# hdelan/MSc-HPC-Final-Project

Hardware: AMD Instinct MI355X
Metric: lanczos_iterations_per_sec (higher is better)
Workload: dtype f64

## Files before the change

### msc-hpc-final-project_amd/csrc/lzx_api.hip

```cpp
#include <algorithm>
#include <atomic>
#include <chrono>
#include <cmath>
#include <cstdlib>
#include <cstring>
#include <string>
#include <thread>

#include "lzx_internal.h"

static thread_local std::string g_err;

void lzx_set_error(const char *fmt, ...)
{
    char buf[1024];
    va_list ap;
    va_start(ap, fmt);
    vsnprintf(buf, sizeof buf, fmt, ap);
    va_end(ap);
    g_err = buf;
}

extern "C" const char *lzx_last_error(void) { return g_err.c_str(); }

// ... 155 lines not shown
}

extern "C" int lzx_test_set_shape(lzx_handle c, const char *name, int64_t value)
{
    if (!c || !name) LZX_FAIL(LZX_ERR_ARG, "lzx_test_set_shape: bad argument");
    if (c->d_row_ptr) LZX_FAIL(LZX_ERR_STATE, "shapes must be set before the graph is handed over");
    const Option *o = find_option(name, OPT_SHAPE);
    if (!o) LZX_FAIL(LZX_ERR_ARG, "lzx_test_set_shape: unknown shape '%s'", name);
    store_option(c, *o, value);
    return LZX_OK;
}

extern "C" int lzx_test_get_shape(lzx_handle c, const char *name, int64_t *value)
{
    if (!c || !name || !value) LZX_FAIL(LZX_ERR_ARG, "lzx_test_get_shape: bad argument");
    if (!strcmp(name, "gather_items_dealt")) *value = c->pb ? c->pb_n_static : 0;
    else if (!strcmp(name, "gather_items_drawn")) *value = c->pb ? c->pb_n_dyn : 0;
    else if (!strcmp(name, "gather_workgroups")) *value = c->pb ? c->pb_gather_grid : 0;
    else if (!strcmp(name, "placement_tried")) *value = c->place_tried;
    else if (!strcmp(name, "placement_kept")) *value = c->place_kept;
    else if (!strcmp(name, "start_vector_was_constant")) *value = c->x0_was_constant ? 1 : 0;
    else if (!strcmp(name, "finish_deferrable")) *value = c->pb && c->pb_defer_ok ? 1 : 0;
    else if (!strcmp(name, "finish_launched")) *value = c->pb && c->pb_finish_grid ? 1 : 0;
    else if (!strncmp(name, "placement_us_", 13) && name[13] >= '0' && name[13] <= '7' && !name[14]) *value = (int64_t)(c->place_ms[name[13] - '0'] * 1e3f);
    else LZX_FAIL(LZX_ERR_ARG, "lzx_test_get_shape: unknown shape '%s'", name);
    return LZX_OK;
}

extern "C" int lzx_test_allreduce_latency(lzx_handle c, uint32_t reps, double *us_each)
{
    if (!c || !us_each || reps == 0) LZX_FAIL(LZX_ERR_ARG, "lzx_test_allreduce_latency: bad argument");
    if (c->comm_kind < 2 || !lzx_exchanges(c)) LZX_FAIL(LZX_ERR_STATE, "lzx_test_allreduce_latency: needs a one-process-per-rank communicator");
    std::vector<lzx_ctx *> cs(1, c);
    LZX_HIP(hipSetDevice(c->device));
    LZX_HIP(hipMemsetAsync(c->d_scal, 0, sizeof(double) * 2, c->stream));
    for (u32 i = 0; i < 5; ++i) LZX_TRY(lzx_comm_allreduce_sum(cs, 0, 2));
    LZX_HIP(hipEventRecord(c->ev_a, c->stream));
    for (u32 i = 0; i < reps; ++i) LZX_TRY(lzx_comm_allreduce_sum(cs, 0, 2));
    LZX_HIP(hipEventRecord(c->ev_b, c->stream));
    LZX_HIP(hipStreamSynchronize(c->stream));
    LZX_TRY(lzx_comm_ipc_check(c));
    float ms = 0.f;
    LZX_HIP(hipEventElapsedTime(&ms, c->ev_a, c->ev_b));
    *us_each = (double)ms * 1e3 / reps;
    return LZX_OK;
}
// ... 1181 lines not shown
```

### msc-hpc-final-project_amd/csrc/lzx_internal.h

```cpp
#pragma once

#include <hip/hip_runtime.h>

#include <algorithm>
#include <chrono>
#include <cmath>
#include <cstdarg>
#include <cstdint>
#include <cstdio>
#include <vector>

#include "lzx.h"

typedef uint32_t u32;
typedef uint64_t u64;

void lzx_set_error(const char *fmt, ...);

#define LZX_HIP(call)                                                                          \
    do {                                                                                       \
        hipError_t e_ = (call);                                                                \
        if (e_ != hipSuccess) {                                                                \
            lzx_set_error("%s:%d: %s -> %s", __FILE__, __LINE__, #call, hipGetErrorString(e_)); \
            return (e_ == hipErrorOutOfMemory) ? LZX_ERR_NOMEM : LZX_ERR_HIP;                   \
// ... 154 lines not shown
    u64 long_elems = 0;
    u32 *d_long_cols = nullptr;
    u64 *d_item_beg = nullptr;
    u32 *d_item_len = nullptr;
    u32 *d_item_first = nullptr;
    double *d_long_partial = nullptr;

    bool pb = false;
    u32 hub_real = 0;
    u64 pb_entries = 0;
    u32 pb_nr = 0;
    u32 pb_units = 0;
    uint16_t *d_pb_lcol = nullptr;
    u32 *d_pb_dst = nullptr;
    uint16_t *d_pb_lrow = nullptr;
    double *d_pb_val = nullptr;
    u32 *d_pb_unit = nullptr;
    u32 *d_pb_row0 = nullptr;
    u32 *d_pb_rep = nullptr;
    u32 *d_pb_beg = nullptr;
    u32 *d_pb_items = nullptr;
    u32 *d_pb_multi = nullptr;
    double *d_pb_part = nullptr;
    uint8_t *d_pb_long_multi = nullptr;
    int64_t pb_stamps_opt = -1;
    unsigned long long *d_pb_gstamps = nullptr;
    int64_t tie_sort_opt = -1;
    int64_t item_opt = -1;
    int64_t vec_per_cu_opt = -1;
    int64_t burst_opt = -1;
    int64_t deep_opt = -1;
    int64_t pb_order_opt = -1;
    int64_t pb_group_opt = -1;
    int64_t pb_group_force_opt = -1;
    int64_t pb_gwaves_opt = -1;
    u32 pb_gather_block = 512;
    u32 pb_n_items = 0, pb_n_multi = 0;
    u32 pb_gather_grid = 0, pb_finish_grid = 0;
    uint4 *d_pb_mrow = nullptr;
    u32 pb_multi_limit = 0;
    bool pb_defer_ok = false, pb_deferring = false;
    int64_t defer_opt = -1;
    double *d_pb_item_dot = nullptr;
    u32 pb_n_static = 0, pb_n_dyn = 0;
    u32 *d_pb_gcounter = nullptr;
    int64_t spmv_wgs_opt = -1;
// ... 318 lines not shown
```

### msc-hpc-final-project_amd/csrc/lzx_kernels.hip

```cpp
#include <type_traits>
#include <algorithm>
#include "lzx_internal.h"
#include "lzx_spmv_body.h"
#include "lzx_reduce.h"


template <int HUB, bool NT>
__global__ void __launch_bounds__(LZX_SPMV_BLOCK) k_spmv(const SpmvArgs a)
{
    spmv_body<HUB, NT>(a, blockIdx.x, gridDim.x);
}

__global__ void __launch_bounds__(LZX_VEC_BLOCK)
k_long_finish(const u32 *item_first, const double *long_partial, u32 n_long, const double *q_loc,
              double *v, double *partials)
{
    __shared__ double sh[4];
    const u32 r = blockIdx.x * LZX_VEC_BLOCK + threadIdx.x;
    double dot = 0.0;
    if (r < n_long) {
        double s = 0.0;
        for (u32 it = item_first[r]; it < item_first[r + 1]; ++it) s += long_partial[it];
        v[r] = s;
        dot = s * q_loc[r];
    }
    block_partial(dot, sh, partials);
}

__global__ void __launch_bounds__(LZX_VEC_BLOCK)
k_reduce(const double *partials, u32 np, double *out, int do_sqrt)
{
    __shared__ double sh[4];
    const double t = block_sum_fixed_256(partials, np, sh);
// ... 445 lines not shown
{
    const u32 need = (c->n_loc_pad / 2 + LZX_VEC_BLOCK - 1) / LZX_VEC_BLOCK;
    const u32 cap = (u32)c->cu_count * (c->vec_per_cu_opt > 0 ? (u32)c->vec_per_cu_opt : (c->n_loc_pad <= (4u << 20) ? 4u : 8u));
    return need < 1 ? 1 : (need < cap ? need : cap);
}

u32 lzx_spmv_partials(const lzx_ctx *c) { return c->spmv_grid + (c->pb ? 0 : c->fin_grid) + lzx_pb_partials(c) - (c->pb_deferring && c->pb_defer_ok ? c->pb_finish_grid : 0u); }

static LazyDeferred lazy_deferred(const lzx_ctx *c)
{
    LazyDeferred d;
    if (c->pb && c->pb_deferring && c->pb_defer_ok) {
        d.mrow = c->d_pb_mrow;
        d.limit = c->pb_multi_limit;
        d.part = c->d_pb_part;
        d.item_first = c->d_item_first;
        d.long_partial = c->d_long_partial;
        d.long_mode = c->d_pb_long_multi;
        d.n_long = c->n_long64;
    }
    return d;
}

template <int HUB, bool NT>
static int launch_spmv_t(lzx_ctx *c, const SpmvArgs &a, hipStream_t st)
{
    auto kern = k_spmv<HUB, NT>;
    LZX_HIP(hipFuncSetAttribute(reinterpret_cast<const void *>(kern),
                                hipFuncAttributeMaxDynamicSharedMemorySize, (int)c->spmv_lds));
    hipLaunchKernelGGL(kern, dim3(c->spmv_grid), dim3(LZX_SPMV_BLOCK), c->spmv_lds, st, a);
    return LZX_OK;
}

int lzx_launch_spmv(lzx_ctx *c, const SpmvLaunch &l)
{
    SpmvArgs a;
    a.sell_cols = c->d_sell_cols;
    a.slice_off = c->d_slice_off;
    a.slice_w = c->d_slice_w;
    const u32 live_slices = l.live_rows_only ? (c->rows_live > c->n_long64 ? (c->rows_live - c->n_long64) / LZX_SLICE : 0u) : c->n_slices;
    a.slice_perm = c->d_slice_perm;
    a.ns_w8 = c->ns_w8;
    a.ns_w4 = c->ns_w4;
    a.ns_w0 = (u32)(std::lower_bound(c->h_slice_w0.begin(), c->h_slice_w0.end(), live_slices) - c->h_slice_w0.begin());
    a.n_slices = c->ns_wide;
    if (c->ns_wide == c->n_slices) a.n_slices = std::min<u32>(c->n_slices, live_slices);
    if (!(c->phase_mask_opt & 2)) a.n_slices = a.ns_w8 = a.ns_w4 = a.ns_w0 = 0;
    a.row0 = c->n_long64;
    a.long_cols = c->d_long_cols;
    a.item_beg = c->d_item_beg;
// ... 19 lines not shown
    if (side) {
        LZX_HIP(hipEventRecord(c->ev_fork, c->stream));
        LZX_HIP(hipStreamWaitEvent(c->stream3, c->ev_fork, 0));
        hs = c->stream3;
    }
    bool fused = false;
    const bool fuse_chunked = c->pb && !side && l.chunk1_ready && c->codes16 && !nt && !c->trace && c->fuse_opt != 0 && c->fuse_opt != 1 &&
                              lzx_pb_can_fuse(c);
    if (fuse_chunked) {
        LZX_TRY(lzx_pb_launch(c, l.x, l.q_loc, l.v, pb_partials, l.chunk1_ready, nullptr, 3, &a, c->spmv_grid, &fused));
        if (fused) {
            LZX_HIP(hipGetLastError());
            return LZX_OK;
        }
        LZX_FAIL(LZX_ERR_STATE, "fused launch was refused");
    }
    if (scatter_first) {
        if (c->trace) LZX_HIP(hipEventRecord(c->trace_ev[2], c->stream));
        const bool fuse = c->codes16 && !nt && !c->trace && c->fuse_opt != 0 && lzx_pb_can_fuse(c);
        LZX_TRY(lzx_pb_launch(c, l.x, l.q_loc, l.v, pb_partials, l.chunk1_ready, nullptr, 1, fuse ? &a : nullptr, c->spmv_grid, &fused));
    }
    if (c->trace) LZX_HIP(hipEventRecord(c->trace_ev[0], c->stream));
    if (fused) {
    } else if (c->codes16) {
        if (nt) LZX_TRY((launch_spmv_t<2, true>(c, a, hs)));
        else    LZX_TRY((launch_spmv_t<2, false>(c, a, hs)));
    } else if (c->hub > 0) {
        if (nt) LZX_TRY((launch_spmv_t<1, true>(c, a, hs)));
        else    LZX_TRY((launch_spmv_t<1, false>(c, a, hs)));
    } else {
        if (nt) LZX_TRY((launch_spmv_t<0, true>(c, a, hs)));
        else    LZX_TRY((launch_spmv_t<0, false>(c, a, hs)));
    }
    if (c->trace) LZX_HIP(hipEventRecord(c->trace_ev[1], c->stream));
    if (c->fin_grid > 0 && !c->pb) {
        hipLaunchKernelGGL(k_long_finish, dim3(c->fin_grid), dim3(LZX_VEC_BLOCK), 0, hs,
                           c->d_item_first, c->d_long_partial, c->n_long64, l.q_loc, l.v,
                           l.partials + c->spmv_grid);
    }
    LZX_HIP(hipGetLastError());
    if (c->trace && !scatter_first) LZX_HIP(hipEventRecord(c->trace_ev[2], c->stream));
    if (side) LZX_HIP(hipEventRecord(c->ev_join, c->stream3));
    if (scatter_first) {
        if (c->trace) LZX_HIP(hipEventRecord(c->trace_ev[5], c->stream));
        LZX_TRY(lzx_pb_launch(c, l.x, l.q_loc, l.v, pb_partials, nullptr, nullptr, 2));
    } else {
// ... 251 lines not shown
```

### msc-hpc-final-project_amd/csrc/lzx_pb.hip

```cpp
#include <hipcub/hipcub.hpp>

#include <algorithm>
#include <cstdlib>
#include <queue>
#include <utility>

#include "lzx_internal.h"
#include "lzx_spmv_body.h"
#include "lzx_pb_shared.h"

namespace {

constexpr u32 KEY_LCOL_BITS = 15, KEY_LROW_SHIFT = KEY_LCOL_BITS, KEY_CBAND_SHIFT = KEY_LROW_SHIFT + 10, KEY_RBAND_SHIFT = KEY_CBAND_SHIFT + 16;
constexpr u32 KEY_LCOL_MASK = (1u << KEY_LCOL_BITS) - 1u;
__device__ __forceinline__ u64 pack_key(u32 rband, u32 cband, u32 lrow, u32 lcol)
{
    return ((u64)rband << KEY_RBAND_SHIFT) | ((u64)cband << KEY_CBAND_SHIFT) | ((u64)lrow << KEY_LROW_SHIFT) | (u64)lcol;
}

__global__ void __launch_bounds__(64)
k_pb_emit(const u64 *row_ptr, const u32 *col_idx, const u32 *code_of_old, const u32 *old_of_local,
          const u32 *deg_local, const u32 *nh_off, u32 n_rows, u32 hub, const u32 *band_row0, u32 nr, u32 cb, u64 *keys)
{
    const u32 lane = threadIdx.x;
    for (u32 l = blockIdx.x; l < n_rows; l += gridDim.x) {
        const u32 d = deg_local[l];
        u32 lo = 0, hi = nr;
        while (hi - lo > 1) {
            const u32 mid = (lo + hi) >> 1;
            if (band_row0[mid] <= l) lo = mid; else hi = mid;
        }
        const u32 R = lo, lrow = l - band_row0[lo];
// ... 481 lines not shown
                    out[1] = hi;
                }
            }
        }
        }
    }
}

template <u32 CB, bool SCAN, bool NTC>
__global__ void __launch_bounds__(1024)
k_pb_scatter(const u32 *unit, const uint4 *scode, const u32 *sbase, const uint2 *q_lcol, const u32 *q_dst,
             const double *__restrict__ x, u64 xlen, double *val)
{
    pb_scatter_body<CB, SCAN, NTC>(unit, scode, sbase, q_lcol, q_dst, x, xlen, val, blockIdx.x);
}

template <u32 CB, bool SCAN, bool NTC>
__global__ void __launch_bounds__(1024)
k_pb_scatter_spmv(const u32 *unit, u32 n_units, const uint4 *scode, const u32 *sbase, const uint2 *q_lcol, const u32 *q_dst,
                  const double *__restrict__ x, u64 xlen, double *val, const SpmvArgs a, const u32 spmv_first)
{
    const u32 spmv_blocks = gridDim.x - n_units;
    if (spmv_first) {
        if (blockIdx.x < spmv_blocks) spmv_body<2, false>(a, blockIdx.x, spmv_blocks);
        else pb_scatter_body<CB, SCAN, NTC>(unit, scode, sbase, q_lcol, q_dst, x, xlen, val, blockIdx.x - spmv_blocks);
        return;
    }
    if (blockIdx.x < n_units) pb_scatter_body<CB, SCAN, NTC>(unit, scode, sbase, q_lcol, q_dst, x, xlen, val, blockIdx.x);
    else spmv_body<2, false>(a, blockIdx.x - n_units, spmv_blocks);
}

template <bool NT>
__device__ __forceinline__ double2 gld_val2(const double *p)
{
    typedef double d2v __attribute__((ext_vector_type(2)));
    const d2v t = NT ? __builtin_nontemporal_load(reinterpret_cast<const d2v *>(p)) : *reinterpret_cast<const d2v *>(p);
    return make_double2(t.x, t.y);
}
template <bool NT>
__device__ __forceinline__ u32 gld_slot2(const uint16_t *p)
{
    return NT ? __builtin_nontemporal_load(reinterpret_cast<const u32 *>(p)) : *reinterpret_cast<const u32 *>(p);
}

__device__ __forceinline__ void tile_add2(double *ytile, u32 lane, u32 sv, double ax, double ay)
{
    const u32 s0 = sv & 0xffffu, s1 = sv >> 16;
    const u32 spare = LZX_PB_RB + lane;
    atomicAdd(&ytile[min(s0, spare)], ax);
    atomicAdd(&ytile[min(s1, spare)], ay);
    if (__ballot((s0 | s1) >= 1024u)) {
        u32 r = 1;
// ... 69 lines not shown
        ticket = uni(*ltick);
        if (ticket >= n_dyn) {
            if (tid == 0 && ticket == n_dyn + gridDim.x - 1) *counter = 0u;
            break;
        }
        base = n_static + ticket; stride = 0; limit = base + 1; nrounds = 1;
        __syncthreads();
    }
    for (u32 t = tid; t < nrounds * WAVES; t += LZX_PB_GATHER_BLOCK) {
        const u32 r = t / WAVES, w = t % WAVES;
        const u32 it = base + r * stride;
        u32 *o = lrec + (size_t)t * 8;
        uint4 item = make_uint4(0u, 0u, 0u, LZX_PB_ITEM_NONE);
        if (it < limit) item = items[it];
        o[5] = item.w;
        o[6] = 0u;
        o[7] = 1u;
        if (item.w == LZX_PB_ITEM_GROUP) {
            const u32 y = item.y, split = y <= 1u ? 8u : y <= 2u ? 4u : y <= 4u ? 2u : 1u;
            o[7] = split;
            if (w < y * split) {
                const u32 R = item.x + w % y;
                const u32 r0 = band_row0[R];
                o[0] = band_beg[R]; o[1] = band_beg[R + 1]; o[2] = r0; o[3] = band_row0[R + 1] - r0; o[4] = band_rep[R]; o[6] = 1u + (w / y) + (y << 8);
            }
        } else if (item.w != LZX_PB_ITEM_NONE) {
            const u32 R = item.x;
            const u32 r0 = band_row0[R];
            o[0] = item.y; o[1] = item.z; o[2] = r0; o[3] = band_row0[R + 1] - r0; o[4] = band_rep[R];
            o[6] = 1u + (item.y == band_beg[R] ? 2u : 0u);
        }
    }
    __syncthreads();
    const double dot_static = dot;
    if (dyn) dot = 0.0;
    for (u32 rr = 0; rr < nrounds && base + rr * stride < limit; ++rr) {
        const u32 *rec = lrec + ((size_t)rr * WAVES + wv) * 8;
        const u32 r_beg = uni(rec[0]), r_end = uni(rec[1]), r_row0 = uni(rec[2]), r_rows = uni(rec[3]), r_rep = uni(rec[4]);
        const u32 item_w = uni(rec[5]), r_live = uni(rec[6]), r_split = uni(rec[7]);
        if (item_w == LZX_PB_ITEM_NONE) continue;
        if (item_w == LZX_PB_ITEM_GROUP) {
            __syncthreads();
            const u32 part = r_live ? (r_live & 0xffu) - 1u : 0u, gy = r_live >> 8;
            if (r_live) {
                const u32 rows = r_rows, rep = r_rep;
                const u32 beg = r_beg, end = r_end;
                const u32 slots = rows * rep;
                for (u32 j = lane; j < slots; j += 64) ytile[j] = 0.0;
                __builtin_amdgcn_wave_barrier();
                if (STAMP && part == 0) { ++n_it; n_vals += end - beg; }
                GSTAMP(t_zero);
                const u32 blocks = (end - beg) / 128u;
                u32 kb = part;
                for (; kb + 7 * r_split < blocks; kb += 8 * r_split) {
                    double2 av[8];
                    u32 sv[8];
#pragma unroll
                    for (int u = 0; u < 8; ++u) {
                        const u32 p = beg + (kb + u * r_split) * 128u + lane * 2;
                        av[u] = gld_val2<NT>(val + p);
                        sv[u] = NOSLOT ? (lane * 2u) | ((lane * 2u + 1u) << 16) : gld_slot2<NT>(lslot + p);
                    }
#pragma unroll
                    for (int u = 0; u < 8; ++u) tile_add2(ytile, lane, sv[u], av[u].x, av[u].y);
                }
                {
// ... 33 lines not shown
                        u32 h8[8];
#pragma unroll
                        for (int u = 0; u < 8; ++u) {
                            h8[u] = ((i + u * 64) * 2654435761u + r_row0 * 40503u) >> 7;
                            t8[u] = xt[h8[u] & 0x1ffffu];
                        }
#pragma unroll
                        for (int u = 0; u < 8; ++u)
                            if (i + u * 64 < probe_l2g) tile_add1(ytile, lane, (h8[u] >> 17) % slots, t8[u]);
                    }
                }
#endif
                __builtin_amdgcn_wave_barrier();
                GSTAMP(t_stream);
            }
            if (r_split > 1u) __syncthreads();
            if (r_live && part == 0u) {
                const u32 row0 = r_row0, rows = r_rows, rep = r_rep;
                for (u32 j0 = lane; j0 < rows; j0 += 256) {
                    double vv[4], qq[4];
#pragma unroll
                    for (int u = 0; u < 4; ++u) {
                        const u32 j = j0 + u * 64;
                        vv[u] = j < rows ? v[row0 + j] : 0.0;
                        qq[u] = j < rows ? q_loc[row0 + j] : 0.0;
                    }
#pragma unroll
                    for (int u = 0; u < 4; ++u) {
                        const u32 j = j0 + u * 64;
                        if (j < rows) {
                            double y = 0.0;
                            for (u32 pt = 0; pt < r_split; ++pt)
                                for (u32 t = 0; t < rep; ++t) y += ytile[(size_t)pt * gy * TILE + j * rep + t];
                            v[row0 + j] = vv[u] + y;
                            dot += y * qq[u];
                        }
                    }
                }
                close_split_rows(row0, rows, lane, 64u, dot, 0u);
                GSTAMP(t_fold);
            }
            continue;
        }
        const u32 beg = r_beg, end = r_end;
        if (STAMP) { ++n_it; n_vals += end - beg; }
        const u32 row0 = r_row0, rows = r_rows;
        if (rows == 1) {
            double acc = 0.0;
            u32 i = beg + tid;
            for (; i + 7 * LZX_PB_GATHER_BLOCK < end; i += 8 * LZX_PB_GATHER_BLOCK) {
                double a[8];
#pragma unroll
                for (int u = 0; u < 8; ++u) a[u] = val[i + u * LZX_PB_GATHER_BLOCK];
#pragma unroll
                for (int u = 0; u < 8; ++u) acc += a[u];
            }
            for (; i < end; i += LZX_PB_GATHER_BLOCK) acc += val[i];
            acc = wave_sum_pb(acc);
            __syncthreads();
            if (lane == 0) wsum[wv] = acc;
            __syncthreads();
            if (tid == 0) {
                double t = 0.0;
                for (u32 w = 0; w < WAVES; ++w) t += wsum[w];
                if (item_w == 0xffffffffu) {
                    double vr = v[row0] + t;
                    dot += t * q_loc[row0];
                    if (row0 < n_long && long_mode[row0] == 0) {
                        double sl = 0.0;
                        for (u32 it = item_first[row0]; it < item_first[row0 + 1]; ++it) sl += long_partial[it];
                        vr += sl;
                        dot += sl * q_loc[row0];
                    }
                    v[row0] = vr;
                } else {
                    part[item_w] = t;
                    dot += t * q_loc[row0];
                    if ((r_live & 2u) && row0 < n_long && long_mode[row0] == 1) {
                        double sl = 0.0;
                        for (u32 it = item_first[row0]; it < item_first[row0 + 1]; ++it) sl += long_partial[it];
                        dot += sl * q_loc[row0];
                    }
                }
            }
            continue;
        }
        const u32 rep = r_rep;
        const u32 slots = rows * rep;
        __syncthreads();
        for (u32 j = lane; j < slots; j += 64) ytile[j] = 0.0;
        __builtin_amdgcn_wave_barrier();
        GSTAMP(t_zero);
        const u32 blocks = (end - beg) / 128u;
        u32 kb = wv;
        for (; kb + 7 * WAVES < blocks; kb += 8 * WAVES) {
            double2 av[8];
            u32 sv[8];
#pragma unroll
            for (int u = 0; u < 8; ++u) {
// ... 4 lines not shown
#pragma unroll
            for (int u = 0; u < 8; ++u) tile_add2(ytile, lane, sv[u], av[u].x, av[u].y);
        }
        for (; kb < blocks; kb += WAVES) {
            const u32 p = beg + kb * 128u + lane * 2;
            const double2 a = gld_val2<NT>(val + p);
            const u32 s = NOSLOT ? (lane * 2u) | ((lane * 2u + 1u) << 16) : gld_slot2<NT>(lslot + p);
            tile_add2(ytile, lane, s, a.x, a.y);
        }
        if (wv == 0)
            for (u32 i0 = beg + blocks * 128u; i0 < end; i0 += 64) {
                const u32 i = i0 + lane;
                tile_add1(ytile, lane, i < end ? (u32)lslot[i] : 0u, i < end ? val[i] : 0.0);
            }
        GSTAMP(t_stream);
        __syncthreads();
        GSTAMP(t_bar);
        if (item_w == 0xffffffffu) {
            for (u32 j0 = tid; j0 < rows; j0 += 2 * LZX_PB_GATHER_BLOCK) {
                double vv[2], qq[2];
#pragma unroll
                for (int u = 0; u < 2; ++u) {
                    const u32 j = j0 + u * LZX_PB_GATHER_BLOCK;
                    vv[u] = j < rows ? v[row0 + j] : 0.0;
                    qq[u] = j < rows ? q_loc[row0 + j] : 0.0;
                }
#pragma unroll
                for (int u = 0; u < 2; ++u) {
                    const u32 j = j0 + u * LZX_PB_GATHER_BLOCK;
                    if (j < rows) {
                        double y = 0.0;
                        for (u32 w = 0; w < WAVES; ++w)
                            for (u32 t = 0; t < rep; ++t) y += lds[(size_t)w * TILE + j * rep + t];
                        v[row0 + j] = vv[u] + y;
                        dot += y * qq[u];
                    }
                }
            }
            close_split_rows(row0, rows, tid, LZX_PB_GATHER_BLOCK, dot, 0u);
        } else {
            for (u32 j = tid; j < rows; j += LZX_PB_GATHER_BLOCK) {
                double y = 0.0;
                for (u32 w = 0; w < WAVES; ++w)
                    for (u32 t = 0; t < rep; ++t) y += lds[(size_t)w * TILE + j * rep + t];
                part[item_w + j] = y;
                dot += y * q_loc[row0 + j];
            }
            if (r_live & 2u) close_split_rows(row0, rows, tid, LZX_PB_GATHER_BLOCK, dot, 1u);
        }
        GSTAMP(t_fold);
    }
    if (dyn) {
        const double idot = wave_sum_pb(dot);
        dot = dot_static;
        __syncthreads();
        if (lane == 0) wsum[wv] = idot;
        __syncthreads();
        if (tid == 0) {
            double t = 0.0;
            for (u32 w = 0; w < WAVES; ++w) t += wsum[w];
            item_dot[ticket] = t;
        }
    } else {
        it0 += MAXR * gridDim.x;
    }
    }
    if (STAMP && tid == 0) {
        unsigned long long *o = stamps + 8 * (size_t)blockIdx.x;
        o[0] = t_start; o[1] = wall_clock64(); o[2] = t_zero; o[3] = t_stream; o[4] = t_bar; o[5] = t_fold;
// ... 102 lines not shown
    LZX_HIP(hipStreamSynchronize(c->stream));
    return rc;
}

void lzx_pb_release(lzx_ctx *c)
{
    pb_free(c->d_pb_lcol);
    pb_free(c->d_pb_dst);
    pb_free(c->d_pb_lrow);
    pb_free(c->d_pb_val);
    pb_free(c->d_pb_unit);
    pb_free(c->d_pb_row0);
    pb_free(c->d_pb_rep);
    pb_free(c->d_pb_beg);
    pb_free(c->d_pb_items);
    pb_free(c->d_pb_gstamps);
    pb_free(c->d_pb_item_dot);
    pb_free(c->d_pb_gcounter);
    pb_free(c->d_pb_multi);
    pb_free(c->d_pb_part);
    pb_free(c->d_pb_long_multi);
    pb_free(c->d_pb_mrow);
    c->pb_multi_limit = 0;
    c->pb_defer_ok = c->pb_deferring = false;
    pb_free(c->d_pbr_code);
    pb_free(c->d_pbr_base);
    c->pb = false;
    c->pb_entries = c->pb_values = c->pbr_entries = 0;
    c->pb_units = c->pb_units0 = c->pb_nr = c->pb_gather_grid = c->pb_n_items = c->pb_n_static = c->pb_n_dyn = c->pb_n_multi = c->pb_finish_grid = 0;
    c->pbr_steps = 0;
}

u32 lzx_pb_partials(const lzx_ctx *c) { return c->pb ? c->pb_gather_grid + c->pb_finish_grid : 0; }

namespace {
struct Arena {
    std::vector<void *> ptrs;
    template <typename T> int get(T **p, u64 count)
    {
        LZX_TRY(pb_alloc(p, count));
        ptrs.push_back(*p);
        return LZX_OK;
    }
    template <typename T> void drop(T *&p)
    {
        for (auto &q : ptrs)
// ... 391 lines not shown
                        u32 R = 0;
                        while (R + 1 < nr && rstart[R + 1] <= i) ++R;
                        fprintf(stderr, "[lzx pb stats]   late value at %llu (band %u begins at %u, offset in band %llu, block offset %llu, rep %u): rows",
                                (unsigned long long)i, R, rstart[R], (unsigned long long)(i - rstart[R]), (unsigned long long)((i - rstart[R]) % 128), rep[R]);
                        for (u64 j = (i >= 6 ? i - 6 : 0); j < std::min<u64>(len, i + 3); ++j) fprintf(stderr, " %s%u/%u", j == i ? "*" : "", (unsigned)hp[j], (unsigned)(hs[j] >> 10));
                        fprintf(stderr, "\n");
                        ++shown;
                    }
            }
            u64 rep1 = 0;
            for (u32 R = 0; R < nr; ++R) rep1 += rep[R] == 1 ? 1 : 0;
            fprintf(stderr, "[lzx pb stats] gather slots: %llu values, %llu of them (%.3f %%) in a round > 0 (highest round %llu), %llu of %llu 128-value blocks (%.2f %%) "
                    "take the slow path; %llu of %u row bands have one slot per row\n", (unsigned long long)len, (unsigned long long)late, 100.0 * late / std::max<double>(1.0, (double)len),
                    (unsigned long long)maxr, (unsigned long long)blocks_late, (unsigned long long)((len + 127) / 128), 100.0 * blocks_late / std::max<double>(1.0, (double)((len + 127) / 128)),
                    (unsigned long long)rep1, nr);
        }
#endif
    }

    std::vector<u32> items, multi;
    u64 slots = 0;
    for (u32 R = 0; R < nr; ++R) {
        const u32 beg = rstart[R], end = rstart[R + 1];
        if (beg == end) continue;
        const u32 rows = row0[R + 1] - row0[R];
        if (end - beg > 2 * target) {
            const u32 cnt = (end - beg + target - 1) / target;
            const u32 piece = ((end - beg + cnt - 1) / cnt + 127u) & ~127u;
            u32 made = 0;
            for (u32 s = beg; s < end; s += piece, ++made) {
                items.push_back(R); items.push_back(s); items.push_back(std::min(end, s + piece));
                items.push_back((u32)(slots + (u64)made * rows));
            }
            for (u32 j = 0; j < rows; ++j) {
                multi.push_back(row0[R] + j); multi.push_back((u32)(slots + j)); multi.push_back(made); multi.push_back(rows);
            }
            slots += (u64)made * rows;
            if (slots >= 0xffffffffull) LZX_FAIL(LZX_ERR_LIMIT, "propagation blocking: item totals overflow 32-bit slots");
        } else {
            items.push_back(R); items.push_back(beg); items.push_back(end); items.push_back(0xffffffffu);
        }
    }
    c->pb_n_items = c->pb_n_static = (u32)(items.size() / 4);
    c->pb_n_dyn = 0;
    c->pb_n_multi = (u32)(multi.size() / 4);
    c->pb_gather_block = c->pb_gwaves_opt == 4 ? 256u : 512u;
    c->pb_gather_grid = std::min<u32>((u32)c->cu_count * (1024u / c->pb_gather_block), std::max(1u, c->pb_n_items));
    if (c->pb_grid_cap_opt > 0) c->pb_gather_grid = std::min<u32>(c->pb_gather_grid, (u32)c->pb_grid_cap_opt);
// ... 68 lines not shown
                    o[0] = it[0]; o[1] = it[1]; o[2] = it[2]; o[3] = it[3];
                } else {
                    o[3] = LZX_PB_ITEM_NONE;
                }
            }
        c->pb_n_static = (u32)(items.size() / 4);
        for (size_t oi = n_dealt; oi < no; ++oi) {
            const u32 *it = &out[4 * (size_t)order[oi]];
            items.insert(items.end(), it, it + 4);
        }
        c->pb_n_dyn = (u32)n_tail;
        c->pb_n_items = (u32)(items.size() / 4);
    }
#ifdef LZX_DEBUG_KNOBS
    if (c->pb_stamps_opt > 0) {
        LZX_TRY(pb_alloc(&c->d_pb_gstamps, 8 * (u64)c->pb_gather_grid));
        LZX_HIP(hipMemsetAsync(c->d_pb_gstamps, 0, sizeof(unsigned long long) * 8 * c->pb_gather_grid, st));
    }
#endif
    u32 n_uncovered = 0;
    {
        std::vector<uint8_t> flag((size_t)c->n_long64 + 1, 2);
        for (u32 R = 0; R < nr; ++R)
            if (rstart[R] != rstart[R + 1])
                for (u32 r = row0[R]; r < std::min<u32>(row0[R + 1], c->n_long64); ++r) flag[r] = 0;
        for (size_t i = 0; i < multi.size(); i += 4)
            if (multi[i] < c->n_long64) flag[multi[i]] = 1;
        for (u32 r = 0; r < c->n_long64; ++r) n_uncovered += flag[r] == 2 ? 1 : 0;
        LZX_TRY(pb_alloc(&c->d_pb_long_multi, flag.size()));
        LZX_HIP(hipMemcpyAsync(c->d_pb_long_multi, flag.data(), flag.size(), hipMemcpyHostToDevice, st));
        LZX_HIP(hipStreamSynchronize(st));
    }
    LZX_TRY(pb_alloc(&c->d_pb_items, items.size())); LZX_TRY(pb_alloc(&c->d_pb_multi, multi.size())); LZX_TRY(pb_alloc(&c->d_pb_part, slots));
    {
        u32 limit = 0;
        for (size_t i = 0; i < multi.size(); i += 4) limit = std::max(limit, multi[i] + 1);
        limit = (limit + 1u) & ~1u;
        std::vector<u32> mrow((size_t)limit * 4, 0u);
        for (size_t i = 0; i < multi.size(); i += 4)
            for (int u = 0; u < 4; ++u) mrow[(size_t)multi[i] * 4 + u] = multi[i + u];
        c->pb_multi_limit = limit;
        LZX_TRY(pb_alloc(&c->d_pb_mrow, (u64)std::max<u32>(limit, 1u)));
        if (limit) LZX_HIP(hipMemcpyAsync(c->d_pb_mrow, mrow.data(), sizeof(u32) * mrow.size(), hipMemcpyHostToDevice, st));
        LZX_HIP(hipStreamSynchronize(st));
    }
    if (!items.empty())
        LZX_HIP(hipMemcpyAsync(c->d_pb_items, items.data(), sizeof(u32) * items.size(), hipMemcpyHostToDevice, st));
    if (!multi.empty())
        LZX_HIP(hipMemcpyAsync(c->d_pb_multi, multi.data(), sizeof(u32) * multi.size(), hipMemcpyHostToDevice, st));

    LZX_TRY(pb_alloc(&c->d_pb_gcounter, 4));
    LZX_HIP(hipMemsetAsync(c->d_pb_gcounter, 0, sizeof(u32) * 4, st));
    if (c->pb_n_dyn) {
        LZX_TRY(pb_alloc(&c->d_pb_item_dot, c->pb_n_dyn));
        LZX_HIP(hipMemsetAsync(c->d_pb_item_dot, 0, sizeof(double) * c->pb_n_dyn, st));
    }
    LZX_TRY(pb_alloc(&c->d_pb_val, len + 8));
    LZX_HIP(hipMemsetAsync(c->d_pb_val, 0, sizeof(double) * (len + 8), st));
    LZX_HIP(hipStreamSynchronize(st));
    LZX_HIP(hipGetLastError());

    c->pb = true;
    c->pb_entries = total;
    c->pbr_entries = red_entries;
    c->pb_values = len;
    c->pb_nr = nr;
    constexpr u32 waves_per_wg = LZX_PB_GATHER_BLOCK / 64;
    (void)waves_per_wg;
    c->pb_finish_grid = (c->pb_n_multi + (n_uncovered ? c->n_long64 : 0u) + LZX_VEC_BLOCK - 1) / LZX_VEC_BLOCK;
    c->pb_defer_ok = c->pb_n_multi > 0 && n_uncovered == 0 && c->pb_n_dyn == 0;
    if (c->pb_n_dyn) c->pb_finish_grid = std::max<u32>(c->pb_finish_grid, (c->pb_n_dyn + LZX_VEC_BLOCK - 1) / LZX_VEC_BLOCK);
    return LZX_OK;
}
#undef GRID
}

int lzx_pb_prepare(lzx_ctx *c, const u32 *d_code, const u32 *d_old_of_local, const u32 *d_deg_local,
                   const u32 *d_nh_off, const std::vector<u32> &h_nh, u64 total)
{
    const int rc = pb_prepare_impl(c, d_code, d_old_of_local, d_deg_local, d_nh_off, h_nh, total);
    if (rc != LZX_OK) {
        (void)hipStreamSynchronize(c->stream);
        lzx_pb_release(c);
    }
// ... 116 lines not shown
```

### msc-hpc-final-project_amd/csrc/lzx_spmv_body.h

```cpp
#pragma once
#include <type_traits>
#include "lzx_internal.h"

__device__ __forceinline__ double wave_sum(double v)
{
#pragma unroll
    for (int o = 32; o > 0; o >>= 1) v += __shfl_xor(v, o, 64);
    return v;
}

struct SpmvArgs {
    const u32 *sell_cols;
    const u64 *slice_off;
    const u32 *slice_w;
    u32 n_slices;
    const u32 *slice_perm;
    u32 ns_w8, ns_w4, ns_w0;
    u32 row0;
    const u32 *long_cols;
    const u64 *item_beg;
    const u32 *item_len;
    u32 n_items;
    double *long_partial;
    const double *x;
// ... 57 lines not shown
}
template <bool NT>
__device__ __forceinline__ uint4 load_raw(const uint4 *p) { return load_idx4<NT>(p); }
template <bool NT>
__device__ __forceinline__ uint2 load_raw(const uint2 *p)
{
#ifdef LZX_ABL_NOLOAD
    return make_uint2((u32)(size_t)p & 0x3fff3fffu, ((u32)(size_t)p >> 3) & 0x3fff3fffu);
#endif
    uint2 r;
    if (NT) {
        r.x = __builtin_nontemporal_load(&p->x);
        r.y = __builtin_nontemporal_load(&p->y);
    } else {
        r = *p;
    }
    return r;
}
__device__ __forceinline__ uint4 codes_of(const uint4 &r) { return r; }
__device__ __forceinline__ uint4 codes_of(const uint2 &r) { return make_uint4(r.x & 0xffffu, r.x >> 16, r.y & 0xffffu, r.y >> 16); }
template <int HUB> struct CodeTable { using packet = uint4; using code = u32; };
template <> struct CodeTable<2> { using packet = uint2; using code = uint16_t; };

template <int HUB, bool NT>
__device__ __forceinline__ void spmv_body(const SpmvArgs &a, const u32 block, const u32 nblocks)
{
    using PK = typename CodeTable<HUB>::packet;
    using CODE = typename CodeTable<HUB>::code;
    const CODE *long_cols = reinterpret_cast<const CODE *>(a.long_cols);
    const CODE *sell_cols = reinterpret_cast<const CODE *>(a.sell_cols);
    extern __shared__ __attribute__((aligned(16))) double lds[];
    double *hubv = lds;
    double *wsum = lds + a.hub;

    const u32 tid = threadIdx.x, lane = tid & 63;
    const u32 wv = (u32)__builtin_amdgcn_readfirstlane((int)(tid >> 6));

    if (HUB) {
        if (!a.burst) {
            for (u32 i = tid; i < a.hub_real; i += LZX_SPMV_BLOCK) {
                const u32 g = (a.world == 1) ? i : (i % a.world) * a.xs0 + i / a.world;
                hubv[i] = a.x[g];
            }
        } else if (a.world == 1) {
            const u32 pairs = a.hub_real >> 1;
            const double2 *src = reinterpret_cast<const double2 *>(a.x);
            auto stage = [&](auto depth_tag) {
// ... 93 lines not shown
                if (j + 1 >= cnt) break;
                issue(j + 2 < cnt ? j + 2 : j + 1, ka);
                consume(j + 1, kb);
            }
        }
    }

    double dot = 0.0;
    {
        const u32 mine = a.n_slices > w0 ? (a.n_slices - w0 + waves - 1) / waves : 0;
        for (u32 base = 0; base < mine; base += 64) {
            const u32 cnt = mine - base < 64 ? mine - base : 64;
            const u32 di = w0 + (base + (lane < cnt ? lane : 0)) * waves;
            const u32 d_sid = a.slice_perm[di];
            const u64 d_off = a.slice_off[d_sid];
            const u32 d_st = a.slice_w[d_sid] >> 2;
            constexpr int PF = 4;
            constexpr int GP = HUB == 2 ? 8 : 4;
            auto issue = [&](u32 j, PK (&f)[PF], double &qrow) {
                const PK *p = reinterpret_cast<const PK *>(sell_cols + lane_u64(d_off, j)) + lane;
                const u32 st = lane_u32(d_st, j);
#pragma unroll
                for (int u = 0; u < PF; ++u) f[u] = load_raw<NT>(p + (size_t)((u32)u < st ? u : 0) * 64);
                qrow = a.q_loc[a.row0 + lane_u32(d_sid, j) * 64 + lane];
            };
            auto add4 = [&](const PK &raw, double &acc) {
                const uint4 k = codes_of(raw);
                const double x0 = gather<HUB>(k.x, a.x, hubv, a.hub);
                const double x1 = gather<HUB>(k.y, a.x, hubv, a.hub);
                const double x2 = gather<HUB>(k.z, a.x, hubv, a.hub);
                const double x3 = gather<HUB>(k.w, a.x, hubv, a.hub);
                acc += x0; acc += x1; acc += x2; acc += x3;
            };
            auto consume = [&](u32 j, const PK (&f)[PF], double qrow) {
                const PK *p = reinterpret_cast<const PK *>(sell_cols + lane_u64(d_off, j)) + lane;
                const u32 st = lane_u32(d_st, j);
                double acc = 0.0;
#pragma unroll
                for (int u = 0; u < PF; ++u)
                    if ((u32)u < st) add4(f[u], acc);
                u32 i = PF;
                for (; i + GP <= st; i += GP) {
                    PK c[GP];
#pragma unroll
                    for (int u = 0; u < GP; ++u) c[u] = load_raw<NT>(p + (size_t)(i + u) * 64);
#pragma unroll
                    for (int u = 0; u < GP; ++u) add4(c[u], acc);
                }
                if (i < st) {
                    PK c[GP - 1];
#pragma unroll
                    for (int u = 0; u < GP - 1; ++u) c[u] = load_raw<NT>(p + (size_t)(i + u < st ? i + u : i) * 64);
#pragma unroll
                    for (int u = 0; u < GP - 1; ++u)
                        if (i + u < st) add4(c[u], acc);
                }
                a.v[a.row0 + lane_u32(d_sid, j) * 64 + lane] = acc;
                dot += acc * qrow;
            };
            if (HUB == 2 && a.deep) {
                PK f0[PF], f1[PF], f2[PF], f3[PF];
                double q0, q1, q2, q3;
                const u32 lastj = cnt - 1;
                auto at = [&](u32 j) { return j < cnt ? j : lastj; };
                issue(0, f0, q0);
                issue(at(1), f1, q1);
                issue(at(2), f2, q2);
                for (u32 j = 0; j < cnt; j += 4) {
                    issue(at(j + 3), f3, q3);
                    consume(j, f0, q0);
                    if (j + 1 >= cnt) break;
                    issue(at(j + 4), f0, q0);
                    consume(j + 1, f1, q1);
                    if (j + 2 >= cnt) break;
                    issue(at(j + 5), f1, q1);
                    consume(j + 2, f2, q2);
                    if (j + 3 >= cnt) break;
                    issue(at(j + 6), f2, q2);
                    consume(j + 3, f3, q3);
                }
            } else {
                PK fa[PF], fb[PF];
                double qa, qb;
                issue(0, fa, qa);
                for (u32 j = 0; j < cnt; j += 2) {
                    issue(j + 1 < cnt ? j + 1 : j, fb, qb);
                    consume(j, fa, qa);
                    if (j + 1 >= cnt) break;
                    issue(j + 2 < cnt ? j + 2 : j + 1, fa, qa);
                    consume(j + 1, fb, qb);
                }
            }
        }
    }

    if (HUB == 2) {
        auto narrow = [&](u32 first, u32 count, auto np_tag) {
            constexpr int NP = decltype(np_tag)::value;
            const u32 mine = count > w0 ? (count - w0 + waves - 1) / waves : 0;
            for (u32 base = 0; base < mine; base += 64) {
                const u32 cnt = mine - base < 64 ? mine - base : 64;
                const u32 d_sid = a.slice_perm[first + w0 + (base + (lane < cnt ? lane : 0)) * waves];
                const u64 d_off = NP ? a.slice_off[d_sid] : 0;
                for (u32 j = 0; j < cnt; j += 4) {
                    PK f[4][NP ? NP : 1];
                    double qr[4];
                    u32 row[4];
#pragma unroll
                    for (int u = 0; u < 4; ++u) {
                        const u32 jj = j + u < cnt ? j + u : cnt - 1;
                        row[u] = a.row0 + lane_u32(d_sid, jj) * 64 + lane;
                        if (NP) {
                            const PK *pp = reinterpret_cast<const PK *>(sell_cols + lane_u64(d_off, jj)) + lane;
#pragma unroll
                            for (int e = 0; e < NP; ++e) f[u][e] = load_raw<NT>(pp + (size_t)e * 64);
                            qr[u] = a.q_loc[row[u]];
                        }
                    }
#pragma unroll
                    for (int u = 0; u < 4; ++u) {
                        if (j + u < cnt) {
                            double acc = 0.0;
#pragma unroll
                            for (int e = 0; e < NP; ++e) {
                                const uint4 k = codes_of(f[u][e]);
                                const double x0 = hubv[k.x], x1 = hubv[k.y], x2 = hubv[k.z], x3 = hubv[k.w];
                                acc += x0; acc += x1; acc += x2; acc += x3;
                            }
                            a.v[row[u]] = acc;
                            if (NP) dot += acc * qr[u];
                        }
                    }
                }
            }
        };
        narrow(a.n_slices, a.ns_w8, std::integral_constant<int, 2>{});
        narrow(a.n_slices + a.ns_w8, a.ns_w4, std::integral_constant<int, 1>{});
        narrow(a.n_slices + a.ns_w8 + a.ns_w4, a.ns_w0, std::integral_constant<int, 0>{});
    }

    dot = wave_sum(dot);
    if (lane == 0) wsum[wv] = dot;
    __syncthreads();
    if (tid == 0) {
        double s = 0.0;
        for (u32 i = 0; i < LZX_SPMV_BLOCK / 64; ++i) s += wsum[i];
        a.partials[block] = s;
    }
}
```

Measured before the change: 1815.

## Move SpMV dot product into PB gather and hand off zero-width slices

```diff
diff --git a/msc-hpc-final-project_amd/csrc/lzx_api.hip b/msc-hpc-final-project_amd/csrc/lzx_api.hip
--- a/msc-hpc-final-project_amd/csrc/lzx_api.hip
+++ b/msc-hpc-final-project_amd/csrc/lzx_api.hip
@@ -201,6 +201,11 @@
     else if (!strcmp(name, "start_vector_was_constant")) *value = c->x0_was_constant ? 1 : 0;
     else if (!strcmp(name, "finish_deferrable")) *value = c->pb && c->pb_defer_ok ? 1 : 0;
     else if (!strcmp(name, "finish_launched")) *value = c->pb && c->pb_finish_grid ? 1 : 0;
+    else if (!strcmp(name, "slices_handed_off")) *value = c->pb ? c->pb_n_handoff : 0;
+    else if (!strcmp(name, "slices_zeroed")) *value = (int64_t)c->h_slice_w0.size();
+    else if (!strcmp(name, "gather_group_items")) *value = c->pb ? c->pb_n_group_items : 0;
+    else if (!strcmp(name, "gather_one_row_items")) *value = c->pb ? c->pb_n_one_row_items : 0;
+    else if (!strcmp(name, "gather_multi_rows")) *value = c->pb ? c->pb_n_multi : 0;
     else if (!strncmp(name, "placement_us_", 13) && name[13] >= '0' && name[13] <= '7' && !name[14]) *value = (int64_t)(c->place_ms[name[13] - '0'] * 1e3f);
     else LZX_FAIL(LZX_ERR_ARG, "lzx_test_get_shape: unknown shape '%s'", name);
     return LZX_OK;
diff --git a/msc-hpc-final-project_amd/csrc/lzx_internal.h b/msc-hpc-final-project_amd/csrc/lzx_internal.h
--- a/msc-hpc-final-project_amd/csrc/lzx_internal.h
+++ b/msc-hpc-final-project_amd/csrc/lzx_internal.h
@@ -200,6 +200,7 @@
     u32 *d_pb_items = nullptr;
     u32 *d_pb_multi = nullptr;
     double *d_pb_part = nullptr;
+    u32 pb_n_handoff = 0, pb_n_group_items = 0, pb_n_one_row_items = 0;
     uint8_t *d_pb_long_multi = nullptr;
     int64_t pb_stamps_opt = -1;
     unsigned long long *d_pb_gstamps = nullptr;
diff --git a/msc-hpc-final-project_amd/csrc/lzx_kernels.hip b/msc-hpc-final-project_amd/csrc/lzx_kernels.hip
--- a/msc-hpc-final-project_amd/csrc/lzx_kernels.hip
+++ b/msc-hpc-final-project_amd/csrc/lzx_kernels.hip
@@ -5,10 +5,10 @@
 #include "lzx_reduce.h"
 
 
-template <int HUB, bool NT>
+template <int HUB, bool NT, bool DOT = true>
 __global__ void __launch_bounds__(LZX_SPMV_BLOCK) k_spmv(const SpmvArgs a)
 {
-    spmv_body<HUB, NT>(a, blockIdx.x, gridDim.x);
+    spmv_body<HUB, NT, DOT>(a, blockIdx.x, gridDim.x);
 }
 
 __global__ void __launch_bounds__(LZX_VEC_BLOCK)
@@ -500,10 +500,10 @@
     return d;
 }
 
-template <int HUB, bool NT>
+template <int HUB, bool NT, bool DOT = true>
 static int launch_spmv_t(lzx_ctx *c, const SpmvArgs &a, hipStream_t st)
 {
-    auto kern = k_spmv<HUB, NT>;
+    auto kern = k_spmv<HUB, NT, DOT>;
     LZX_HIP(hipFuncSetAttribute(reinterpret_cast<const void *>(kern),
                                 hipFuncAttributeMaxDynamicSharedMemorySize, (int)c->spmv_lds));
     hipLaunchKernelGGL(kern, dim3(c->spmv_grid), dim3(LZX_SPMV_BLOCK), c->spmv_lds, st, a);
@@ -569,6 +569,9 @@
     }
     if (c->trace) LZX_HIP(hipEventRecord(c->trace_ev[0], c->stream));
     if (fused) {
+    } else if (c->codes16 && c->pb) {
+        if (nt) LZX_TRY((launch_spmv_t<2, true, false>(c, a, hs)));
+        else    LZX_TRY((launch_spmv_t<2, false, false>(c, a, hs)));
     } else if (c->codes16) {
         if (nt) LZX_TRY((launch_spmv_t<2, true>(c, a, hs)));
         else    LZX_TRY((launch_spmv_t<2, false>(c, a, hs)));
diff --git a/msc-hpc-final-project_amd/csrc/lzx_pb.hip b/msc-hpc-final-project_amd/csrc/lzx_pb.hip
--- a/msc-hpc-final-project_amd/csrc/lzx_pb.hip
+++ b/msc-hpc-final-project_amd/csrc/lzx_pb.hip
@@ -8,6 +8,7 @@
 #include "lzx_internal.h"
 #include "lzx_spmv_body.h"
 #include "lzx_pb_shared.h"
+#include "lzx_pb_handoff.h"
 
 namespace {
 
@@ -535,12 +536,12 @@
 {
     const u32 spmv_blocks = gridDim.x - n_units;
     if (spmv_first) {
-        if (blockIdx.x < spmv_blocks) spmv_body<2, false>(a, blockIdx.x, spmv_blocks);
+        if (blockIdx.x < spmv_blocks) spmv_body<2, false, false>(a, blockIdx.x, spmv_blocks);
         else pb_scatter_body<CB, SCAN, NTC>(unit, scode, sbase, q_lcol, q_dst, x, xlen, val, blockIdx.x - spmv_blocks);
         return;
     }
     if (blockIdx.x < n_units) pb_scatter_body<CB, SCAN, NTC>(unit, scode, sbase, q_lcol, q_dst, x, xlen, val, blockIdx.x);
-    else spmv_body<2, false>(a, blockIdx.x - n_units, spmv_blocks);
+    else spmv_body<2, false, false>(a, blockIdx.x - n_units, spmv_blocks);
 }
 
 template <bool NT>
@@ -656,13 +657,15 @@
             if (w < y * split) {
                 const u32 R = item.x + w % y;
                 const u32 r0 = band_row0[R];
-                o[0] = band_beg[R]; o[1] = band_beg[R + 1]; o[2] = r0; o[3] = band_row0[R + 1] - r0; o[4] = band_rep[R]; o[6] = 1u + (w / y) + (y << 8);
+                o[0] = band_beg[R]; o[1] = band_beg[R + 1]; o[2] = r0; const u32 rw = band_rep[R];
+                o[3] = band_row0[R + 1] - r0; o[4] = rw & 0xffffu; o[6] = (1u + (w / y) + (y << 8)) | (rw & 0xffff0000u);
             }
         } else if (item.w != LZX_PB_ITEM_NONE) {
             const u32 R = item.x;
             const u32 r0 = band_row0[R];
-            o[0] = item.y; o[1] = item.z; o[2] = r0; o[3] = band_row0[R + 1] - r0; o[4] = band_rep[R];
-            o[6] = 1u + (item.y == band_beg[R] ? 2u : 0u);
+            o[0] = item.y; o[1] = item.z; o[2] = r0; const u32 rw = band_rep[R];
+            o[3] = band_row0[R + 1] - r0; o[4] = rw & 0xffffu;
+            o[6] = (1u + (item.y == band_beg[R] ? 2u : 0u)) | (rw & 0xffff0000u);
         }
     }
     __syncthreads();
@@ -672,10 +675,11 @@
         const u32 *rec = lrec + ((size_t)rr * WAVES + wv) * 8;
         const u32 r_beg = uni(rec[0]), r_end = uni(rec[1]), r_row0 = uni(rec[2]), r_rows = uni(rec[3]), r_rep = uni(rec[4]);
         const u32 item_w = uni(rec[5]), r_live = uni(rec[6]), r_split = uni(rec[7]);
+        const u32 w0m = r_live >> 16;
         if (item_w == LZX_PB_ITEM_NONE) continue;
         if (item_w == LZX_PB_ITEM_GROUP) {
             __syncthreads();
-            const u32 part = r_live ? (r_live & 0xffu) - 1u : 0u, gy = r_live >> 8;
+            const u32 part = r_live ? (r_live & 0xffu) - 1u : 0u, gy = (r_live >> 8) & 0xffu;
             if (r_live) {
                 const u32 rows = r_rows, rep = r_rep;
                 const u32 beg = r_beg, end = r_end;
@@ -755,7 +759,7 @@
 #pragma unroll
                     for (int u = 0; u < 4; ++u) {
                         const u32 j = j0 + u * 64;
-                        vv[u] = j < rows ? v[row0 + j] : 0.0;
+                        vv[u] = (j < rows && !((w0m >> (j >> 6)) & 1u)) ? v[row0 + j] : 0.0;
                         qq[u] = j < rows ? q_loc[row0 + j] : 0.0;
                     }
 #pragma unroll
@@ -766,6 +770,7 @@
                             for (u32 pt = 0; pt < r_split; ++pt)
                                 for (u32 t = 0; t < rep; ++t) y += ytile[(size_t)pt * gy * TILE + j * rep + t];
                             v[row0 + j] = vv[u] + y;
+                            dot += vv[u] * qq[u];
                             dot += y * qq[u];
                         }
                     }
@@ -797,7 +802,9 @@
                 double t = 0.0;
                 for (u32 w = 0; w < WAVES; ++w) t += wsum[w];
                 if (item_w == 0xffffffffu) {
-                    double vr = v[row0] + t;
+                    const double vs = (w0m & 1u) ? 0.0 : v[row0];
+                    double vr = vs + t;
+                    dot += vs * q_loc[row0];
                     dot += t * q_loc[row0];
                     if (row0 < n_long && long_mode[row0] == 0) {
                         double sl = 0.0;
@@ -808,6 +815,10 @@
                     v[row0] = vr;
                 } else {
                     part[item_w] = t;
+                    if (r_live & 2u) {
+                        if (w0m & 1u) v[row0] = 0.0;
+                        else dot += v[row0] * q_loc[row0];
+                    }
                     dot += t * q_loc[row0];
                     if ((r_live & 2u) && row0 < n_long && long_mode[row0] == 1) {
                         double sl = 0.0;
@@ -858,7 +869,7 @@
 #pragma unroll
                 for (int u = 0; u < 2; ++u) {
                     const u32 j = j0 + u * LZX_PB_GATHER_BLOCK;
-                    vv[u] = j < rows ? v[row0 + j] : 0.0;
+                    vv[u] = (j < rows && !((w0m >> (j >> 6)) & 1u)) ? v[row0 + j] : 0.0;
                     qq[u] = j < rows ? q_loc[row0 + j] : 0.0;
                 }
 #pragma unroll
@@ -869,6 +880,7 @@
                         for (u32 w = 0; w < WAVES; ++w)
                             for (u32 t = 0; t < rep; ++t) y += lds[(size_t)w * TILE + j * rep + t];
                         v[row0 + j] = vv[u] + y;
+                        dot += vv[u] * qq[u];
                         dot += y * qq[u];
                     }
                 }
@@ -880,7 +892,12 @@
                 for (u32 w = 0; w < WAVES; ++w)
                     for (u32 t = 0; t < rep; ++t) y += lds[(size_t)w * TILE + j * rep + t];
                 part[item_w + j] = y;
-                dot += y * q_loc[row0 + j];
+                const double qj = q_loc[row0 + j];
+                if (r_live & 2u) {
+                    if ((w0m >> (j >> 6)) & 1u) v[row0 + j] = 0.0;
+                    else dot += v[row0 + j] * qj;
+                }
+                dot += y * qj;
             }
             if (r_live & 2u) close_split_rows(row0, rows, tid, LZX_PB_GATHER_BLOCK, dot, 1u);
         }
@@ -1029,6 +1046,7 @@
     pb_free(c->d_pb_long_multi);
     pb_free(c->d_pb_mrow);
     c->pb_multi_limit = 0;
+    c->pb_n_handoff = c->pb_n_group_items = c->pb_n_one_row_items = 0;
     c->pb_defer_ok = c->pb_deferring = false;
     pb_free(c->d_pbr_code);
     pb_free(c->d_pbr_base);
@@ -1466,8 +1484,8 @@
     u64 slots = 0;
     for (u32 R = 0; R < nr; ++R) {
         const u32 beg = rstart[R], end = rstart[R + 1];
-        if (beg == end) continue;
         const u32 rows = row0[R + 1] - row0[R];
+        if (rows == 0) continue;
         if (end - beg > 2 * target) {
             const u32 cnt = (end - beg + target - 1) / target;
             const u32 piece = ((end - beg + cnt - 1) / cnt + 127u) & ~127u;
@@ -1582,8 +1600,7 @@
     {
         std::vector<uint8_t> flag((size_t)c->n_long64 + 1, 2);
         for (u32 R = 0; R < nr; ++R)
-            if (rstart[R] != rstart[R + 1])
-                for (u32 r = row0[R]; r < std::min<u32>(row0[R + 1], c->n_long64); ++r) flag[r] = 0;
+            for (u32 r = row0[R]; r < std::min<u32>(row0[R + 1], c->n_long64); ++r) flag[r] = 0;
         for (size_t i = 0; i < multi.size(); i += 4)
             if (multi[i] < c->n_long64) flag[multi[i]] = 1;
         for (u32 r = 0; r < c->n_long64; ++r) n_uncovered += flag[r] == 2 ? 1 : 0;
@@ -1620,6 +1637,22 @@
     LZX_HIP(hipStreamSynchronize(st));
     LZX_HIP(hipGetLastError());
 
+    {
+        std::vector<u32> w0mask, kept;
+        lzx_pb_handoff(row0, c->n_long64, c->h_slice_w0, w0mask, kept);
+        for (u32 R = 0; R < nr; ++R) w0mask[R] = rep[R] | (w0mask[R] << 16);
+        LZX_HIP(hipMemcpyAsync(c->d_pb_rep, w0mask.data(), sizeof(u32) * nr, hipMemcpyHostToDevice, st));
+        if (!kept.empty())
+            LZX_HIP(hipMemcpyAsync(c->d_slice_perm + (c->ns_wide + c->ns_w8 + c->ns_w4), kept.data(), sizeof(u32) * kept.size(), hipMemcpyHostToDevice, st));
+        LZX_HIP(hipStreamSynchronize(st));
+        c->h_slice_w0.swap(kept);
+        c->pb_n_handoff = (u32)(kept.size() - c->h_slice_w0.size());
+        c->pb_n_group_items = c->pb_n_one_row_items = 0;
+        for (size_t i = 0; i + 3 < items.size(); i += 4) {
+            if (items[i + 3] == LZX_PB_ITEM_GROUP) ++c->pb_n_group_items;
+            else if (items[i + 3] != LZX_PB_ITEM_NONE && row0[items[i] + 1] - row0[items[i]] == 1) ++c->pb_n_one_row_items;
+        }
+    }
     c->pb = true;
     c->pb_entries = total;
     c->pbr_entries = red_entries;
diff --git a/msc-hpc-final-project_amd/csrc/lzx_pb_handoff.h b/msc-hpc-final-project_amd/csrc/lzx_pb_handoff.h
--- /dev/null
+++ b/msc-hpc-final-project_amd/csrc/lzx_pb_handoff.h
@@ -0,0 +1,38 @@
+#pragma once
+#include <algorithm>
+#include <cstdint>
+#include <vector>
+
+static inline void lzx_pb_handoff(const std::vector<uint32_t> &row0, uint32_t body_row0, const std::vector<uint32_t> &w0,
+                                  std::vector<uint32_t> &mask, std::vector<uint32_t> &kept)
+{
+    constexpr uint32_t G = 64;
+    const uint32_t nr = row0.empty() ? 0u : (uint32_t)row0.size() - 1u;
+    const uint32_t band_end = nr ? row0[nr] : 0u;
+    auto slice_is_w0 = [&](uint32_t s) { return std::binary_search(w0.begin(), w0.end(), s); };
+    auto rows_are_w0 = [&](uint32_t a, uint32_t b) {
+        if (a >= b || a < body_row0) return false;
+        for (uint32_t s = (a - body_row0) / G; s <= (b - 1u - body_row0) / G; ++s)
+            if (!slice_is_w0(s)) return false;
+        return true;
+    };
+    mask.assign(nr, 0u);
+    for (uint32_t R = 0; R < nr; ++R) {
+        const uint32_t rows = row0[R + 1] - row0[R];
+        if (rows > 16u * G) continue;
+        for (uint32_t g = 0; g * G < rows; ++g)
+            if (rows_are_w0(row0[R] + g * G, row0[R] + std::min(rows, (g + 1u) * G))) mask[R] |= 1u << g;
+    }
+    kept.clear();
+    for (uint32_t s : w0) {
+        const uint64_t lo = (uint64_t)body_row0 + (uint64_t)s * G, hi = lo + G;
+        bool off = nr > 0 && hi <= band_end;
+        for (uint64_t r = lo; off && r < hi;) {
+            const uint32_t R = (uint32_t)(std::upper_bound(row0.begin(), row0.begin() + nr + 1, (uint32_t)r) - row0.begin()) - 1u;
+            const uint32_t g = ((uint32_t)r - row0[R]) / G;
+            off = g < 16u && ((mask[R] >> g) & 1u);
+            r = std::min<uint64_t>(row0[R + 1], (uint64_t)row0[R] + (uint64_t)(g + 1u) * G);
+        }
+        if (!off) kept.push_back(s);
+    }
+}
diff --git a/msc-hpc-final-project_amd/csrc/lzx_spmv_body.h b/msc-hpc-final-project_amd/csrc/lzx_spmv_body.h
--- a/msc-hpc-final-project_amd/csrc/lzx_spmv_body.h
+++ b/msc-hpc-final-project_amd/csrc/lzx_spmv_body.h
@@ -103,7 +103,7 @@
 template <int HUB> struct CodeTable { using packet = uint4; using code = u32; };
 template <> struct CodeTable<2> { using packet = uint2; using code = uint16_t; };
 
-template <int HUB, bool NT>
+template <int HUB, bool NT, bool DOT = true>
 __device__ __forceinline__ void spmv_body(const SpmvArgs &a, const u32 block, const u32 nblocks)
 {
     using PK = typename CodeTable<HUB>::packet;
@@ -243,7 +243,7 @@
                 const u32 st = lane_u32(d_st, j);
 #pragma unroll
                 for (int u = 0; u < PF; ++u) f[u] = load_raw<NT>(p + (size_t)((u32)u < st ? u : 0) * 64);
-                qrow = a.q_loc[a.row0 + lane_u32(d_sid, j) * 64 + lane];
+                if (DOT) qrow = a.q_loc[a.row0 + lane_u32(d_sid, j) * 64 + lane];
             };
             auto add4 = [&](const PK &raw, double &acc) {
                 const uint4 k = codes_of(raw);
@@ -277,11 +277,11 @@
                         if (i + u < st) add4(c[u], acc);
                 }
                 a.v[a.row0 + lane_u32(d_sid, j) * 64 + lane] = acc;
-                dot += acc * qrow;
+                if (DOT) dot += acc * qrow;
             };
             if (HUB == 2 && a.deep) {
                 PK f0[PF], f1[PF], f2[PF], f3[PF];
-                double q0, q1, q2, q3;
+                double q0 = 0.0, q1 = 0.0, q2 = 0.0, q3 = 0.0;
                 const u32 lastj = cnt - 1;
                 auto at = [&](u32 j) { return j < cnt ? j : lastj; };
                 issue(0, f0, q0);
@@ -302,7 +302,7 @@
                 }
             } else {
                 PK fa[PF], fb[PF];
-                double qa, qb;
+                double qa = 0.0, qb = 0.0;
                 issue(0, fa, qa);
                 for (u32 j = 0; j < cnt; j += 2) {
                     issue(j + 1 < cnt ? j + 1 : j, fb, qb);
@@ -325,7 +325,7 @@
                 const u64 d_off = NP ? a.slice_off[d_sid] : 0;
                 for (u32 j = 0; j < cnt; j += 4) {
                     PK f[4][NP ? NP : 1];
-                    double qr[4];
+                    double qr[4] = {0.0, 0.0, 0.0, 0.0};
                     u32 row[4];
 #pragma unroll
                     for (int u = 0; u < 4; ++u) {
@@ -335,7 +335,7 @@
                             const PK *pp = reinterpret_cast<const PK *>(sell_cols + lane_u64(d_off, jj)) + lane;
 #pragma unroll
                             for (int e = 0; e < NP; ++e) f[u][e] = load_raw<NT>(pp + (size_t)e * 64);
-                            qr[u] = a.q_loc[row[u]];
+                            if (DOT) qr[u] = a.q_loc[row[u]];
                         }
                     }
 #pragma unroll
@@ -349,7 +349,7 @@
                                 acc += x0; acc += x1; acc += x2; acc += x3;
                             }
                             a.v[row[u]] = acc;
-                            if (NP) dot += acc * qr[u];
+                            if (NP && DOT) dot += acc * qr[u];
                         }
                     }
                 }
@@ -360,6 +360,10 @@
         narrow(a.n_slices + a.ns_w8 + a.ns_w4, a.ns_w0, std::integral_constant<int, 0>{});
     }
 
+    if (!DOT) {
+        if (tid == 0) a.partials[block] = 0.0;
+        return;
+    }
     dot = wave_sum(dot);
     if (lane == 0) wsum[wv] = dot;
     __syncthreads();
```

New measurement: 1832, median of 6. Within noise of the previous version (+0.9%).
